# syncdoth/face_mask_inpaint

Measured on AMD Instinct MI355X. Metric: train images/sec at 256x256 bs=8 per GPU (PICNet-ref train step), higher is better.
Workload: dtype f32; 1 GPU; train_reference_fill.py PICNet-ref 256x256 fp32, bs=8 per GPU, synthetic CelebA-HQ-shaped batch + random binary_map (BASELINE configs[1]); global_batch=8, parallelism=dp1

## Files before the change

face_mask_inpaint_amd/_lib.py:

```python
from __future__ import annotations

import ctypes as C
import os

_HERE = os.path.dirname(os.path.abspath(__file__))
LIB_PATH = os.path.join(_HERE, "csrc", "libfmi_hip.so")

c_f = C.c_void_p
i32, i64, f32, vp = C.c_int, C.c_int64, C.c_float, C.c_void_p


class ConvDesc(C.Structure):

    _fields_ = [(n, C.c_int) for n in ("N", "H", "W", "C", "OH", "OW", "K", "x_cstride", "y_cstride", "kh", "kw", "stride", "pad", "pad_mode", "dil")] + [("w3", C.c_void_p), ("x3", C.c_void_p), ("y3", C.c_void_p)]


class WeightEntry(C.Structure):
    _fields_ = [("w", vp), ("u", vp), ("v", vp), ("wf", vp), ("wt", vp), ("sigma", vp), ("rows", i32), ("C", i32), ("taps", i32), ("iters", i32), ("wf3", vp), ("wt3", vp)]


class WeightGradEntry(C.Structure):
    _fields_ = [("w", vp), ("u", vp), ("v", vp), ("sigma", vp), ("dwf", vp), ("dw", vp), ("rows", i32), ("C", i32), ("taps", i32), ("pad_", i32)]


# ... 82 lines not shown
    "fmi_add_bcast_f32": [vp, vp, vp, i32, i64, i32, vp],
    "fmi_scale_channels_bwd_f32": [vp, vp, vp, vp, vp, vp, i64, i32, i64, i32, vp],
    "fmi_subsample_bf16": [vp, vp, i32, i32, i32, i32, i32, i32, vp],
    "fmi_scale_channels_add_f32": [vp, vp, vp, vp, i32, i64, i32, vp],
    "fmi_instnorm_bwd_apply_add_f32": [vp, vp, vp, vp, vp, vp, vp, vp, vp, vp, i32, i32, i32, f32, vp],
    "fmi_copy_channels_f32": [vp, vp, i64, i32, i32, i32, i32, i32, vp],
    "fmi_l2norm_rows_f32": [vp, vp, vp, i64, i32, f32, vp],
    "fmi_l2norm_rows_bwd_f32": [vp, vp, vp, vp, i64, i32, f32, vp],
    "fmi_lpips_layer_f32": [vp, vp, vp, vp, i64, i32, f32, vp],
    "fmi_lpips_layer_bwd_f32": [vp, vp, vp, vp, vp, vp, i64, i32, f32, vp],
    "fmi_maxpool2_bwd_f32": [vp, vp, vp, i32, i32, i32, i32, vp],
    "fmi_resize_bilinear_f32": [vp, vp, i32, i32, i32, i32, i32, i32, vp, vp, vp],
    "fmi_resize_bilinear_bwd_f32": [vp, vp, i32, i32, i32, i32, i32, i32, vp, vp],
    "fmi_instnorm_stats_f32": [vp, vp, vp, i32, i32, i32, f32, vp, i64, vp],
    "fmi_batchnorm_running_update_f32": [vp, vp, vp, vp, vp, i32, i64, f32, f32, vp],
    "fmi_instnorm_apply_f32": [vp, vp, vp, vp, vp, i32, i32, i32, f32, vp],
    "fmi_instnorm_bwd_reduce_f32": [vp, vp, vp, vp, vp, vp, i32, i32, i32, f32, vp, i64, vp],
    "fmi_instnorm_bwd_apply_f32": [vp, vp, vp, vp, vp, vp, vp, vp, vp, i32, i32, i32, f32, vp],
    "fmi_reduce_loss_f32": [i32, vp, vp, i64, f32, f32, vp, vp],
    "fmi_reduce_loss_bwd_f32": [i32, vp, vp, i64, f32, f32, vp, vp, vp],
    "fmi_ssim_f32": [vp, vp, vp, i32, i32, i32, i32, i32, vp, vp],
    "fmi_cx_channel_mean_f32": [vp, vp, i64, i32, vp],
    "fmi_cx_normalise_f32": [vp, vp, vp, vp, i64, i32, vp],
    "fmi_cx_normalise_bwd_f32": [vp, vp, vp, vp, i64, i32, vp],
    "fmi_cx_rows_f32": [vp, vp, vp, vp, vp, i32, i32, f32, vp],
    "fmi_cx_cols_f32": [vp, vp, vp, i32, i32, vp],
    "fmi_cx_loss_f32": [vp, vp, vp, i32, i32, f32, vp],
    "fmi_cx_bwd_f32": [vp, vp, vp, vp, vp, vp, vp, vp, vp, i32, i32, f32, f32, vp],
    "fmi_adam_step_f32": [vp, i32, i64, f32, f32, f32, f32, f32, i32, vp],
    "fmi_adam_step_dev_f32": [vp, i32, f32, f32, f32, f32, f32, vp, vp],
    "fmi_adam_step_dev_guarded_f32": [vp, i32, f32, f32, f32, f32, f32, vp, vp, vp],
    "fmi_ranger_step_f32": [vp, i32, f32, f32, f32, f32, f32, f32, i32, f32, i32, vp],
    "fmi_upfirdn2d_f32": [vp, vp, vp, i32, i32, i32, i32, i32, i32, i32, i32, i32, i32, i32, i32, i32, vp],
    "fmi_upfirdn2d_bf16": [vp, vp, vp, i32, i32, i32, i32, i32, i32, i32, i32, i32, i32, i32, i32, i32, vp],
    "fmi_fused_bias_act_f32": [vp, vp, vp, vp, i64, i32, i32, i32, i32, f32, f32, vp],
    "fmi_fused_bias_act_bf16": [vp, vp, vp, vp, i64, i32, i32, i32, i32, f32, f32, vp],
    "fmi_scale_channels_f32": [vp, vp, vp, i32, i64, i32, vp],
    "fmi_scale_channels_gs_f32": [vp, vp, vp, vp, i64, i32, i64, i32, vp],
    "fmi_sqsum_last_f32": [vp, vp, i64, i32, vp],
    "fmi_sqsum_last_bwd_f32": [vp, vp, vp, i64, i32, vp],
    "fmi_noise_bias_act_bwd_f32": [vp, vp, vp, vp, vp, i64, i32, f32, f32, vp],
    "fmi_upfirdn2d_nhwc_f32": [vp, vp, vp, i32, i32, i32, i32, i32, i32, i32, i32, i32, i32, i32, i32, i32, i32, vp],
    "fmi_prelu_f32": [vp, vp, vp, i64, i32, vp],
    "fmi_prelu_bwd_f32": [vp, vp, vp, vp, vp, vp, i64, i64, i32, vp],
    "fmi_subsample_f32": [vp, vp, i32, i32, i32, i32, i32, i32, vp],
    "fmi_bias_grad_nchw_f32": [vp, i32, i32, i64, vp, vp],
    "fmi_bias_grad_nchw_bf16": [vp, i32, i32, i64, vp, vp],
    "fmi_noise_bias_act_f32": [vp, vp, vp, vp, vp, i64, i32, f32, f32, vp],
}

STATUS = {0: "ok", 1: "bad argument", 2: "unsupported shape/mode", 3: "kernel launch failed"}


PREDICATES = {"fmi_debug_bf16_tile": [i32], "fmi_set_deterministic": [i32], "fmi_get_deterministic": [], "fmi_conv2d_thin_supported": [PD], "fmi_conv2d_bf16_supported": [PD], "fmi_conv2d_thin_lrelu_supported": [PD]}


class FmiError(RuntimeError):
    pass


class Library:

    def __init__(self, path: str = LIB_PATH, strict: bool = True):
        if not os.path.exists(path):
            raise FmiError(
                f"{path} not found: build the HIP extension first (python -c 'import __graft_entry__ as g; g.build()'). "
                "There is no CPU fallback."
            )
        self.path = path
        self.cdll = C.CDLL(path)
        self.missing = []
        for name, argtypes in SIGNATURES.items():
            try:
                fn = getattr(self.cdll, name)
            except AttributeError:
                self.missing.append(name)
                continue
            fn.argtypes = argtypes
            fn.restype = C.c_int
            setattr(self, name[4:], self._checked(name, fn))
        for name, argtypes in PREDICATES.items():
            try:
                fn = getattr(self.cdll, name)
            except AttributeError:
                self.missing.append(name)
                continue
            fn.argtypes = argtypes
            fn.restype = C.c_int
            setattr(self, name[4:], fn)
        if strict and self.missing:
            raise FmiError(f"{path} lacks symbols {self.missing}")

    @staticmethod
    def _checked(name, fn):
        def call(*args):
            rc = fn(*args)
            if rc != 0:
                raise FmiError(f"{name} failed: {STATUS.get(rc, rc)}")

        call.__name__ = name
        return call


_LIB = None


def lib() -> Library:
# ... 5 lines not shown
```

face_mask_inpaint_amd/csrc/conv.hip:

```cpp
#include "gemm_core.h"
#include "conv3x3.h"
#include "conv_p3.h"
#include "convt3x3.h"

static bool aligned16(const void* p) { return ((uintptr_t)p & 15) == 0; }
static bool ep_scalar() {
  static const bool v = getenv("FMI_EP_SCALAR") != nullptr;
  return v;
}

static int check_desc(const fmi_conv_desc* d) {
  if (!d) return FMI_ERR_BAD_ARG;
  if (d->N <= 0 || d->H <= 0 || d->W <= 0 || d->C <= 0 || d->K <= 0 || d->kh <= 0 || d->kw <= 0 || d->stride <= 0 ||
      d->pad < 0 || d->x_cstride < d->C || d->y_cstride < d->K)
    return FMI_ERR_BAD_ARG;
  const int pe = d->pad, dl = d->dil > 1 ? d->dil : 1;
  if (d->dil < 0 || (dl > 1 && d->pad_mode)) return FMI_ERR_BAD_ARG;
  if (d->OH != (d->H + 2 * pe - dl * (d->kh - 1) - 1) / d->stride + 1 || d->OW != (d->W + 2 * pe - dl * (d->kw - 1) - 1) / d->stride + 1)
    return FMI_ERR_BAD_ARG;
  if (d->OH <= 0 || d->OW <= 0) return FMI_ERR_BAD_ARG;
  if (d->pad_mode == 1 && (d->pad >= d->H || d->pad >= d->W)) return FMI_ERR_UNSUPPORTED;
  if (d->pad_mode != 0 && d->pad_mode != 1) return FMI_ERR_UNSUPPORTED;
  if ((int64_t)d->N * d->H * d->W > 0x7fffffffLL / 2 || (int64_t)d->kh * d->kw * d->C > 0x3fffffffLL) return FMI_ERR_UNSUPPORTED;
  return FMI_OK;
}

static ConvGeom fwd_geom(const fmi_conv_desc* d, const float* x, int n_eff) {
  ConvGeom g{};
  g.N = n_eff; g.IH = d->H; g.IW = d->W; g.C = d->C; g.cstride = d->x_cstride;
  g.GH = d->OH; g.GW = d->OW; g.S = d->stride;
  const int dl = d->dil > 1 ? d->dil : 1;
  g.nty = d->kh; g.ntx = d->kw; g.dy0 = -d->pad; g.dx0 = -d->pad; g.ystep = dl; g.xstep = dl;
  g.kh0 = 0; g.kw0 = 0; g.khstep = 1; g.kwstep = 1; g.kw = d->kw;
  g.pad_mode = d->pad_mode;
  g.vec = (d->C % 4 == 0) && (d->x_cstride % 4 == 0) && aligned16(x);
  g.dGW = make_fastdiv(g.GW); g.dG = make_fastdiv(g.GH * g.GW); g.dC = make_fastdiv(g.C); g.dntx = make_fastdiv(g.ntx);
  g.img_bs = (int64_t)d->H * d->W * d->x_cstride;
  return g;
}

#ifndef FMI_HOST_EMU
__global__ void __launch_bounds__(256) conv_split_init_kernel(float* __restrict__ y, const float* __restrict__ bias,
                                                             const float* __restrict__ res, int K, int cstride, int64_t total) {
  for (int64_t i = (int64_t)blockIdx.x * 256 + threadIdx.x; i < total; i += (int64_t)gridDim.x * 256) {
    const int k = (int)(i % K);
    const int64_t o = (i / K) * cstride + k;
    float v = bias ? bias[k] : 0.f;
    if (res) v += res[o];
    y[o] = v;
  }
}
#endif

static int conv_ksplit(int64_t M, int N, int K) {
#ifdef FMI_HOST_EMU
  return 1;
// ... 296 lines not shown
        continue;
      }
#endif
      rc = launch_gemm(la, lb, ep, g.Mdim(), d->C, g.Kdim(), batch_w, 1, (hipStream_t)stream);
      if (rc) return rc;
    }
  }
  return FMI_OK;
}
extern "C" int fmi_conv2d_dgrad_f32(const fmi_conv_desc* d, const float* dy, const float* wt, const float* bias,
                                    const float* residual, float* dx, int batch_w, int64_t w_bstride, void* stream) {
  return dgrad_impl(d, dy, wt, bias, residual, nullptr, 0.f, dx, batch_w, w_bstride, stream);
}
extern "C" int fmi_conv_transpose2d_pair_f32(const fmi_conv_desc* d, const float* x1, const float* x2, int K2, const void* w3b,
                                             const float* bias, float* y, void* stream) {
  int rc = check_desc(d);
  if (rc) return rc;
  if (!x1 || !x2 || !w3b || !d->w3 || !y || K2 <= 0) return FMI_ERR_BAD_ARG;
#ifndef FMI_HOST_EMU
  const uint16_t* w3 = (FMI_X6 && d->K % 16 == 0 && aligned16(d->w3)) ? (const uint16_t*)d->w3 : nullptr;
  if (!convt3x3_eligible(d, x1, w3) || (K2 & 15) || !aligned16(x2) || !aligned16(w3b) || d->pad_mode != 0 || d->x3) return FMI_ERR_UNSUPPORTED;
  CT3Args ca{};
  ca.x = x1; ca.w3 = w3; ca.x2 = x2; ca.w3b = (const uint16_t*)w3b; ca.Cred2 = K2; ca.cs2 = K2;
  ca.N = d->N; ca.H = d->OH; ca.W = d->OW; ca.Cred = d->K; ca.cs = d->y_cstride; ca.Nout = d->C;
  ca.dW = make_fastdiv(d->OW); ca.dHW = make_fastdiv(d->OH * d->OW);
  ConvEp ep{y, bias, nullptr, d->OH, d->OW, 2, 0, 0, d->H, d->W, d->x_cstride, 0, ca.dW, ca.dHW, (int64_t)d->H * d->W * d->x_cstride};
  ep.vec = !ep_scalar() && d->C % 4 == 0 && d->x_cstride % 4 == 0 && aligned16(y) && aligned16(bias);
  ca.ep = ep;
  return launch_convt3x3(ca, d->N * d->OH * d->OW, (hipStream_t)stream);
#else
  return FMI_ERR_UNSUPPORTED;
#endif
}
extern "C" int fmi_conv2d_dgrad_masked_f32(const fmi_conv_desc* d, const float* dy, const float* wt, const float* mask, float mask_slope,
                                           float* dx, void* stream) {
  if (!mask) return FMI_ERR_BAD_ARG;
  return dgrad_impl(d, dy, wt, nullptr, nullptr, mask, mask_slope, dx, 1, 0, stream);
}

extern "C" int fmi_conv2d_dgrad_masked_add_f32(const fmi_conv_desc* d, const float* dy, const float* wt, const float* mask, float mask_slope,
                                               const float* gadd, float* dx, void* stream) {
  if (!mask || !gadd) return FMI_ERR_BAD_ARG;
  return dgrad_impl(d, dy, wt, nullptr, gadd, mask, mask_slope, dx, 1, 0, stream);
}

extern "C" int fmi_conv2d_wgrad_f32(const fmi_conv_desc* d, const float* x, const float* dy, float* dwf, float* dbias,
                                    int batch_w, int64_t w_bstride, void* stream) {
  int rc = check_desc(d);
  if (rc) return rc;
  if (!x || !dy || !dwf || batch_w < 1) return FMI_ERR_BAD_ARG;
  if (batch_w > 1 && batch_w != d->N) return FMI_ERR_BAD_ARG;
#ifndef FMI_HOST_EMU
  if (batch_w == 1 && fmi_conv2d_thin_supported(d) && aligned16(x)) return fmi_conv2d_thin_wgrad_f32(d, x, dy, dwf, dbias, stream);
#endif
#ifndef FMI_HOST_EMU
  static const bool wg3_off = getenv("FMI_WG3_OFF") != nullptr || getenv("FMI_P3_OFF") != nullptr;
  if (!wg3_off && FMI_X6 && batch_w == 1 && !dbias && wgrad_p3_ok(d, d->x3, d->y3))
    return launch_wgrad_p3(d, (const uint16_t*)d->x3, (const uint16_t*)d->y3, dwf, (hipStream_t)stream);
#endif
  const int n_eff = batch_w > 1 ? 1 : d->N;
  ConvGeom g = fwd_geom(d, x, n_eff);
  const bool fuse_bias = dbias && batch_w == 1 && (g.Kdim() % 4 == 0);
  if (dbias && !fuse_bias) return FMI_ERR_UNSUPPORTED;
  const int ones_row = fuse_bias ? g.Kdim() : -1;
  const int Mg = g.Kdim() + (fuse_bias ? 1 : 0), Ng = d->K, Kg = g.Mdim();
  WgradAX la{x, g, ones_row};
  DenseX lb{dy, (int64_t)d->y_cstride, (int64_t)d->OH * d->OW * d->y_cstride, Ng, Kg,
            (d->K % 4 == 0) && (d->y_cstride % 4 == 0) && aligned16(dy)};
  WgradEp ep{dwf, g, d->K, w_bstride, dbias, ones_row};
  const int64_t tiles = ceil_div64(Mg, 128) * ceil_div64(Ng, Ng <= 32 ? 32 : (Ng <= 64 ? 64 : 128));
  int64_t ksplit = 2048 / (tiles * batch_w);
  const int64_t kmax = Kg / 512;
  if (ksplit > kmax) ksplit = kmax;
  if (ksplit < 1) ksplit = 1;
  static const int wks_dbg = getenv("FMI_WKS") ? atoi(getenv("FMI_WKS")) : 0;
  if (wks_dbg > 0) ksplit = wks_dbg;
  if (fmi_det()) ksplit = 1;
  if (ksplit * batch_w > 65535) ksplit = 65535 / batch_w;
  return launch_gemm(la, lb, ep, Mg, Ng, Kg, batch_w, (int)ksplit, (hipStream_t)stream);
}

#ifndef FMI_HOST_EMU
__global__ void __launch_bounds__(256) bias_grad_vec_f64_kernel(const float* __restrict__ g, int64_t rows, int K4, float* __restrict__ dbias) {
  __shared__ double part[256][4];
  const int cg = threadIdx.x % K4, rl = threadIdx.x / K4, RL = 256 / K4;
  double s[4] = {0, 0, 0, 0};
  for (int64_t r = rl; r < rows; r += RL) {
    const float4 v = reinterpret_cast<const float4*>(g)[r * K4 + cg];
    s[0] += v.x, s[1] += v.y, s[2] += v.z, s[3] += v.w;
  }
#pragma unroll
  for (int e = 0; e < 4; ++e) part[threadIdx.x][e] = s[e];
  __syncthreads();
  if (threadIdx.x < K4) {
    double t[4] = {0, 0, 0, 0};
    for (int l = 0; l < RL; ++l)
#pragma unroll
      for (int e = 0; e < 4; ++e) t[e] += part[l * K4 + threadIdx.x][e];
#pragma unroll
    for (int e = 0; e < 4; ++e) atomicAdd(dbias + 4 * threadIdx.x + e, (float)t[e]);
  }
}
__global__ void __launch_bounds__(256) bias_grad_vec_kernel(const float* __restrict__ g, int64_t rows, int K4,
                                                            float* __restrict__ dbias, int64_t rows_per_block) {
  __shared__ float4 part[256];
  const int cg = threadIdx.x % K4, rl = threadIdx.x / K4, RL = 256 / K4;
  const int64_t r0 = (int64_t)blockIdx.x * rows_per_block;
  int64_t r1 = r0 + rows_per_block;
  if (r1 > rows) r1 = rows;
  float4 s = make_float4(0.f, 0.f, 0.f, 0.f);
  int64_t r = r0 + rl;
  for (; r + 3 * RL < r1; r += 4 * RL) {
    const float4 v0 = reinterpret_cast<const float4*>(g)[r * K4 + cg];
    const float4 v1 = reinterpret_cast<const float4*>(g)[(r + RL) * K4 + cg];
    const float4 v2 = reinterpret_cast<const float4*>(g)[(r + 2 * RL) * K4 + cg];
    const float4 v3 = reinterpret_cast<const float4*>(g)[(r + 3 * RL) * K4 + cg];
    s.x += (v0.x + v1.x) + (v2.x + v3.x);
    s.y += (v0.y + v1.y) + (v2.y + v3.y);
    s.z += (v0.z + v1.z) + (v2.z + v3.z);
    s.w += (v0.w + v1.w) + (v2.w + v3.w);
  }
  for (; r < r1; r += RL) {
    const float4 v = reinterpret_cast<const float4*>(g)[r * K4 + cg];
    s.x += v.x; s.y += v.y; s.z += v.z; s.w += v.w;
  }
  part[threadIdx.x] = s;
  __syncthreads();
  if (threadIdx.x < K4) {
    float4 t = part[threadIdx.x];
    for (int l = 1; l < RL; ++l) {
      const float4 v = part[l * K4 + threadIdx.x];
      t.x += v.x; t.y += v.y; t.z += v.z; t.w += v.w;
// ... 76 lines not shown
```

face_mask_inpaint_amd/functional.py:

```python
from __future__ import annotations

import ctypes as C
import math
import os
from typing import List, Optional, Sequence, Tuple

import torch

from . import _lib
from ._lib import ConvDesc, FmiError

EW_LRELU, EW_LRELU_BWD, EW_TANH_BWD, EW_ADD, EW_SCALE, EW_AXPY, EW_MUL, EW_RELU_BWD_OUT, EW_SOFTPLUS, EW_SOFTPLUS_BWD, EW_SUB, EW_RSQRT, EW_RSQRT_BWD, EW_SIGMOID, EW_SIGMOID_BWD = range(15)
ACT_NONE, ACT_TANH, ACT_RELU = 0, 1, 2

ATTN_CHUNK_BYTES = 96 * 1024 * 1024

PROFILE = None


class _prof:
    def __init__(self, tag, flops):
        self.tag, self.flops = tag, flops

    def __enter__(self):
# ... 293 lines not shown
        if gy is None:
            return (gpass,) + (None,) * 15
        kh, kw, stride, pad, pad_mode, act = ctx.cfg
        gy = gy.contiguous()
        if act and not ctx.skip_act_bwd:
            gy = _act_bwd(gy, y, act)
        n, h, w, c = x.shape
        k = wf.shape[2]
        gx = gwf = gb = gres = None
        masked = False
        dil = ctx.dil
        gb_of_split = [] if (ctx.has[0] and ctx.needs_input_grad[2]) else None
        if ctx.needs_input_grad[0]:
            d0, _, _ = conv_desc(n, h, w, c, k, kh, kw, stride, pad, pad_mode, dil=dil)
            if pad_mode == 1 and lib.conv2d_thin_supported(C.byref(d0)):
                gx = torch.empty_like(x)
                with _prof(f"conv_dgrad|{n}x{h}x{w} {c}->{k} k{kh}s{stride}", 2.0 * gy.numel() * c * kh * kw):
                    lib.conv2d_thin_dgrad_f32(C.byref(d0), _p(gy), _p(ctx.wt), _p(gx), _st())
            elif pad_mode == 1:
                hp, wp = h + 2 * pad, w + 2 * pad
                d, _, _ = conv_desc(n, hp, wp, c, k, kh, kw, stride, 0, w3=ctx.wt3)
                gpad = torch.empty((n, hp, wp, c), device=x.device, dtype=torch.float32)
                with _prof(f"conv_dgrad|{n}x{h}x{w} {c}->{k} k{kh}s{stride}", 2.0 * gy.numel() * c * kh * kw):
                    lib.conv2d_dgrad_f32(C.byref(d), _p(gy), _p(ctx.wt), None, None, _p(gpad), 1, 0, _st())
                gx = torch.empty_like(x)
                lib.reflect_pad_fold_f32(_p(gpad), _p(gx), n, h, w, c, pad, _st())
            else:
                oh_, ow_ = gy.shape[1], gy.shape[2]
                gy3 = p3_of(gy, colsum=gb_of_split) if (ctx.wt3 is not None and p3_wanted(n * oh_ * ow_, k, c, kh * kw)) else None
                d, _, _ = conv_desc(n, h, w, c, k, kh, kw, stride, pad, dil=dil, w3=ctx.wt3, x3=gy3)
                gx = torch.empty_like(x)
                with _prof(f"conv_dgrad|{n}x{h}x{w} {c}->{k} k{kh}s{stride}", 2.0 * gy.numel() * c * kh * kw):
                    if ctx.in_slope is not None and gpass is not None:
                        lib.conv2d_dgrad_masked_add_f32(C.byref(d), _p(gy), _p(ctx.wt), _p(x), ctx.in_slope, _p(gpass.contiguous()), _p(gx), _st())
                        masked, gpass = True, None
                    elif ctx.in_slope is not None:
                        lib.conv2d_dgrad_masked_f32(C.byref(d), _p(gy), _p(ctx.wt), _p(x), ctx.in_slope, _p(gx), _st())
                        masked = True
                    elif gpass is not None:
                        lib.conv2d_dgrad_f32(C.byref(d), _p(gy), _p(ctx.wt), None, _p(gpass.contiguous()), _p(gx), 1, 0, _st())
                        gpass = None
                    else:
                        lib.conv2d_dgrad_f32(C.byref(d), _p(gy), _p(ctx.wt), None, None, _p(gx), 1, 0, _st())
            if ctx.in_slope is not None and not masked:
                gx = eltwise(EW_LRELU_BWD, gx, x, ctx.in_slope)
            if gpass is not None:
                gx = eltwise(EW_ADD, gx, gpass.contiguous())
        elif gpass is not None:
            gx = gpass
        if ctx.needs_input_grad[1]:
            d, _, _ = conv_desc(n, h, w, c, k, kh, kw, stride, pad, pad_mode, dil=dil)
            gwf = _zeros_like(wf)
            want_gb = ctx.has[0] and ctx.needs_input_grad[2]
            if ctx.x3 is not None and pad_mode == 0 and c % 32 == 0 and k % 16 == 0 and p3_wanted(gy.numel() // k, c, k, kh * kw):
                gy3 = p3_of(gy, colsum=gb_of_split)
                if gy3 is not None:
                    d.w3 = None
                    d.x3, d.y3 = ctx.x3.data_ptr(), gy3.data_ptr()
                    want_gb_fused = False
                else:
                    want_gb_fused = want_gb
            else:
                want_gb_fused = want_gb
            fuse = want_gb_fused and (kh * kw * c) % 4 == 0
            if fuse:
                gb = _zeros(k, x.device, torch.float32)
            with _prof(f"conv_wgrad|{n}x{h}x{w} {c}->{k} k{kh}s{stride}", 2.0 * gy.numel() * c * kh * kw):
                lib.conv2d_wgrad_f32(C.byref(d), _p(x), _p(gy), _p(gwf), _p(gb) if fuse else None, 1, 0, _st())
        if ctx.has[0] and ctx.needs_input_grad[2] and gb is None:
            if gb_of_split:
                gb = gb_of_split[0]
            else:
                gb = _zeros(k, x.device, torch.float32)
                lib.bias_grad_f32(_p(gy), gy.numel() // k, k, k, _p(gb), _st())
        if ctx.has[1] and ctx.needs_input_grad[3]:
            gres = gy
        return gx, gwf, gb, gres, None, None, None, None, None, None, None, None, None, None, None, None


class _ThinConvLReLU(torch.autograd.Function):

    @staticmethod
    def forward(ctx, x, wf, bias, wt, slope, pad_mode, act):
        _chk(x, wf, bias)
        n, h, w, c = x.shape
        k = wf.shape[2]
        d, oh, ow = conv_desc(n, h, w, c, k, 3, 3, 1, 1, pad_mode)
        y = torch.empty((n, oh, ow, k), device=x.device, dtype=torch.float32)
        with _prof(f"conv_fwd|{n}x{h}x{w} {c}->{k} k3s1", 2.0 * n * oh * ow * k * c * 9):
            _L().conv2d_thin_lrelu_fwd_f32(C.byref(d), _p(x), slope, _p(wf), _p(bias), _p(y), act, _st())
        ctx.save_for_backward(x, wf, y if act else None)
        ctx.wt, ctx.cfg, ctx.has_b = wt, (slope, pad_mode, act), bias is not None
        return y

    @staticmethod
    def backward(ctx, gy):
        lib = _L()
        x, wf, y = ctx.saved_tensors
        slope, pad_mode, act = ctx.cfg
        gy = gy.contiguous()
        if act:
            gy = _act_bwd(gy, y, act)
        n, h, w, c = x.shape
        k = wf.shape[2]
        d, _, _ = conv_desc(n, h, w, c, k, 3, 3, 1, 1, pad_mode)
        gx = gwf = gb = None
        if ctx.needs_input_grad[0]:
# ... 282 lines not shown
def _bias_grad_of(gy, cb):
    m = _BIAS_GRAD_MEMO
    if m[0] is not None and m[0].data_ptr() == gy.data_ptr() and m[0].shape == gy.shape and m[0]._version == gy._version and m[2] == gy._version:
        return m[1].clone()
    gb = _zeros(cb, gy.device, torch.float32)
    _L().bias_grad_f32(_p(gy), gy.numel() // cb, cb, cb, _p(gb), _st())
    m[:] = [gy, gb, gy._version]
    return gb.clone()


class _ConvTranspose2d(torch.autograd.Function):

    @staticmethod
    def forward(ctx, x, wf, bias, residual, wt, kh, kw, stride, pad, out_pad, w3=(None, None)):
        _chk(x, wf, bias, residual)
        lib = _L()
        n, h, w, cs = x.shape
        cb = wf.shape[1]
        H = (h - 1) * stride - 2 * pad + kh + out_pad
        W = (w - 1) * stride - 2 * pad + kw + out_pad
        x3 = p3_of(x) if (w3[1] is not None and p3_wanted(n * h * w, cs, cb, kh * kw)) else None
        d, oh, ow = conv_desc(n, H, W, cb, cs, kh, kw, stride, pad, w3=w3[1], x3=x3)
        ctx.wf3 = w3[0]
        ctx.x3 = x3
        if (oh, ow) != (h, w):
            raise FmiError("unsupported ConvTranspose2d geometry")
        y = torch.empty((n, H, W, cb), device=x.device, dtype=torch.float32)
        with _prof(f"convT_fwd|{n}x{h}x{w} {cs}->{cb}", 2.0 * x.numel() * cb * kh * kw):
            lib.conv2d_dgrad_f32(C.byref(d), _p(x), _p(wt), _p(bias), _p(residual), _p(y), 1, 0, _st())
        ctx.save_for_backward(x, wf)
        ctx.cfg, ctx.has, ctx.HW = (kh, kw, stride, pad), (bias is not None, residual is not None), (H, W)
        return y

    @staticmethod
    def backward(ctx, gy):
        lib = _L()
        x, wf = ctx.saved_tensors
        kh, kw, stride, pad = ctx.cfg
        H, W = ctx.HW
        gy = gy.contiguous()
        n, h, w, cs = x.shape
        cb = wf.shape[1]
        d, _, _ = conv_desc(n, H, W, cb, cs, kh, kw, stride, pad, w3=ctx.wf3)
        gx = gwf = gb = gres = None
        gb_of_split = [] if (ctx.has[0] and ctx.needs_input_grad[2]) else None
        if ctx.needs_input_grad[0]:
            gx = torch.empty_like(x)
            gy3 = p3_of(gy, colsum=gb_of_split) if (ctx.wf3 is not None and p3_wanted(n * H * W, cb, cs, kh * kw)) else None
            d0, _, _ = conv_desc(n, H, W, cb, cs, kh, kw, stride, pad, w3=ctx.wf3, x3=gy3)
            with _prof(f"convT_dgrad|{n}x{h}x{w} {cs}->{cb}", 2.0 * x.numel() * cb * kh * kw):
                lib.conv2d_fwd_f32(C.byref(d0), _p(gy), _p(wf), None, None, _p(gx), 0, 1, 0, _st())
        if ctx.needs_input_grad[1]:
            gwf = _zeros_like(wf)
            if ctx.x3 is not None and cb % 32 == 0 and cs % 16 == 0:
                gy3 = p3_of(gy, colsum=gb_of_split)
                if gy3 is not None:
                    d.x3, d.y3 = gy3.data_ptr(), ctx.x3.data_ptr()
            with _prof(f"convT_wgrad|{n}x{h}x{w} {cs}->{cb}", 2.0 * x.numel() * cb * kh * kw):
                lib.conv2d_wgrad_f32(C.byref(d), _p(gy), _p(x), _p(gwf), None, 1, 0, _st())
        if ctx.has[0] and ctx.needs_input_grad[2]:
            gb = gb_of_split[0] if gb_of_split else _bias_grad_of(gy, cb)
        if ctx.has[1] and ctx.needs_input_grad[3]:
            gres = gy
        return gx, gwf, gb, gres, None, None, None, None, None, None, None


class _ConvTransposePair(torch.autograd.Function):

    @staticmethod
    def forward(ctx, x1, wf1, wt1, x2, wf2, wt2, bias, w3_1, w3_2):
        _chk(x1, wf1, x2, wf2, bias)
        n, h, w, cs1 = x1.shape
        cs2, cb = x2.shape[3], wf1.shape[1]
        H, W = 2 * h, 2 * w
        d, oh, ow = conv_desc(n, H, W, cb, cs1, 3, 3, 2, 1, w3=w3_1[1])
        y = torch.empty((n, H, W, cb), device=x1.device, dtype=torch.float32)
        with _prof(f"convT_pair_fwd|{n}x{h}x{w} {cs1}+{cs2}->{cb}", 2.0 * (x1.numel() + x2.numel()) * cb * 9):
            _L().conv_transpose2d_pair_f32(C.byref(d), _p(x1), _p(x2), cs2, C.c_void_p(w3_2[1].data_ptr()), _p(bias), _p(y), _st())
        ctx.save_for_backward(x1, wf1, x2, wf2)
        ctx.w3s, ctx.HW, ctx.has_bias = (w3_1, w3_2), (H, W), bias is not None
        return y

    @staticmethod
    def backward(ctx, gy):
        import types

        x1, wf1, x2, wf2 = ctx.saved_tensors
        gy = gy.contiguous()
        outs = []
        for x, wf, w3, ix, iw in ((x1, wf1, ctx.w3s[0], 0, 1), (x2, wf2, ctx.w3s[1], 3, 4)):
            ns = types.SimpleNamespace(saved_tensors=(x, wf), cfg=(3, 3, 2, 1), has=(False, False), HW=ctx.HW, wf3=w3[0], x3=None,
                                       needs_input_grad=(ctx.needs_input_grad[ix], ctx.needs_input_grad[iw]) + (False,) * 9)
            outs.append(_ConvTranspose2d.backward(ns, gy)[:2])
        gb = _bias_grad_of(gy, gy.shape[-1]) if (ctx.has_bias and ctx.needs_input_grad[6]) else None
        return outs[0][0], outs[0][1], None, outs[1][0], outs[1][1], None, gb, None, None


def conv_transpose2d_pair_ok(x1, pw1: PackedWeight, x2, pw2: PackedWeight) -> bool:
    if x1.dtype != torch.float32 or x2.dtype != torch.float32 or not x1.is_cuda or x1.shape[:3] != x2.shape[:3]:
        return False
    if os.environ.get("FMI_CT3_OFF"):
        return False
    n, h, w, cs1 = x1.shape
    cs2, cb = x2.shape[3], pw1.wf.shape[1]
    return (pw1.kh == 3 and pw1.kw == 3 and pw2.kh == 3 and pw2.kw == 3 and pw2.wf.shape[1] == cb and cb <= 64 and cb % 4 == 0 and cs1 % 16 == 0 and
            cs2 % 16 == 0 and n * h * w >= 32768 and pw1.w3[1] is not None and pw2.w3[1] is not None and x1.is_contiguous() and x2.is_contiguous() and
            not p3_wanted(n * h * w, cs1, cb, 9))
# ... 1356 lines not shown
```

include/fmi_hip.h:

```cpp
#ifndef FMI_HIP_H
#define FMI_HIP_H

#include <stdint.h>

#ifdef __cplusplus
extern "C" {
#endif

typedef enum {
  FMI_OK = 0,
  FMI_ERR_BAD_ARG = 1,
  FMI_ERR_UNSUPPORTED = 2,
  FMI_ERR_LAUNCH = 3
} fmi_status;

const char* fmi_status_string(int status);
int fmi_version(void);
int fmi_set_deterministic(int on);
int fmi_get_deterministic(void);

int fmi_debug_bf16_tile(int mode);

int fmi_gemm_f32(const float* A, const float* B, float* C, int M, int N, int K,
                 int64_t sa_m, int64_t sa_k, int64_t sb_k, int64_t sb_n, int64_t sc_m, int64_t sc_n,
                 int batch, int64_t sa_b, int64_t sb_b, int64_t sc_b,
                 float alpha, float beta, const float* bias, void* stream);

typedef struct {
  int N, H, W, C;
  int OH, OW, K;
  int x_cstride;
  int y_cstride;
  int kh, kw, stride, pad;
  int pad_mode;
  int dil;
  const void* w3;
  const void* x3;
  void* y3;
} fmi_conv_desc;

int fmi_resample_u8(const uint8_t* in, uint8_t* out, int N, int in_h, int in_w, int C, int out_len, int axis, int row0, int rows,
                    const int32_t* bounds, const int32_t* kk, int ksize, void* stream);
int fmi_gather_u8_i64(const uint8_t* in, int64_t* out, int N, int in_h, int in_w, int out_h, int out_w, const int32_t* ytab,
                      const int32_t* xtab, void* stream);
int fmi_u8_lut_chw_f32(const uint8_t* in, const float* lut256, float* out, int N, int H, int W, int C, void* stream);

int fmi_split3_f32(const float* x, void* x3, float* y, int64_t pixels, int C, int op, float p0, void* stream);
int fmi_merge3_f32(const void* x3, float* y, int64_t pixels, int C, void* stream);
int fmi_split3_colsum_f32(const float* x, void* x3, float* colsum, int64_t pixels, int C, void* stream);

int fmi_conv2d_fwd_f32(const fmi_conv_desc* d, const float* x, const float* wf, const float* bias,
                       const float* residual, float* y, int act, int batch_w, int64_t w_bstride, void* stream);
int fmi_conv_transpose2d_pair_f32(const fmi_conv_desc* d, const float* x1, const float* x2, int K2, const void* w3b, const float* bias,
                                  float* y, void* stream);
int fmi_conv2d_dgrad_f32(const fmi_conv_desc* d, const float* dy, const float* wt, const float* bias,
                         const float* residual, float* dx, int batch_w, int64_t w_bstride, void* stream);
int fmi_conv2d_dgrad_masked_f32(const fmi_conv_desc* d, const float* dy, const float* wt, const float* mask, float mask_slope, float* dx,
                                void* stream);
int fmi_conv2d_dgrad_masked_add_f32(const fmi_conv_desc* d, const float* dy, const float* wt, const float* mask, float mask_slope,
                                    const float* gadd, float* dx, void* stream);
int fmi_conv2d_wgrad_f32(const fmi_conv_desc* d, const float* x, const float* dy, float* dwf, float* dbias,
                         int batch_w, int64_t w_bstride, void* stream);
int fmi_conv2d_thin_supported(const fmi_conv_desc* d);
int fmi_conv2d_thin_fwd_f32(const fmi_conv_desc* d, const float* x, const float* wf, const float* bias,
                            const float* residual, float* y, int act, void* stream);
int fmi_conv2d_thin_dgrad_f32(const fmi_conv_desc* d, const float* dy, const float* wt, float* dx, void* stream);
int fmi_conv2d_thin_wgrad_f32(const fmi_conv_desc* d, const float* x, const float* dy, float* dwf, float* dbias, void* stream);
int fmi_conv2d_thin_lrelu_supported(const fmi_conv_desc* d);
int fmi_conv2d_thin_lrelu_fwd_f32(const fmi_conv_desc* d, const float* x, float in_slope, const float* wf, const float* bias, float* y, int act,
                                  void* stream);
int fmi_conv2d_thin_lrelu_dgrad_f32(const fmi_conv_desc* d, const float* dy, const float* wt, const float* x, float in_slope, float* dx,
                                    void* stream);
int fmi_conv2d_thin_lrelu_wgrad_f32(const fmi_conv_desc* d, const float* x, float in_slope, const float* dy, float* dwf, float* dbias,
                                    void* stream);
int fmi_conv2d_thin_input_dgrad_f32(const fmi_conv_desc* d, const float* dy, const float* wt, float* dx, void* stream);
int fmi_conv2d_bf16_supported(const fmi_conv_desc* d);
int fmi_conv2d_fwd_bf16(const fmi_conv_desc* d, const uint16_t* x, const uint16_t* wnk, const float* colscale, uint16_t* y, float* ws,
                        int64_t ws_floats, void* stream);
int fmi_conv2d_fwd_act_bf16(const fmi_conv_desc* d, const uint16_t* x, const uint16_t* wnk, const float* colscale, const float* noise,
                            const float* nw, const float* bias, float slope, float gain, uint16_t* y, void* stream);
int fmi_conv2d_dgrad_bf16(const fmi_conv_desc* d, const uint16_t* dy, const uint16_t* wck, const float* colscale, uint16_t* dx, float* ws,
                          int64_t ws_floats, void* stream);
int fmi_conv2d_wgrad_bf16(const fmi_conv_desc* d, const uint16_t* x, const uint16_t* dy, float* dwf, void* stream);
int fmi_pack_weight_bf16(const float* src_tab, uint16_t* dst_bta, int T, int A, int B, void* stream);
int fmi_scale_channels_bf16(const uint16_t* x, const float* s, uint16_t* y, int N, int64_t P, int C, void* stream);
int fmi_scale_channels_gs_bf16(const uint16_t* g, const uint16_t* x, float* gs, float* ws, int64_t ws_floats, int N, int64_t P, int C,
                               void* stream);
int fmi_noise_bias_act_bf16(const uint16_t* x, const float* bias, const float* noise, const float* nw, uint16_t* y, int64_t pixels, int C,
                            float alpha, float scale, void* stream);
int fmi_noise_bias_act_bwd_bf16(const uint16_t* g, const uint16_t* y, const float* noise, uint16_t* gx, float* gnw, float* gbias,
                                float* ws, int64_t ws_floats, int64_t pixels, int C, float alpha, float scale, void* stream);
int fmi_upfirdn2d_nhwc_bf16(const uint16_t* in, const float* kernel, uint16_t* out, int N, int in_h, int in_w, int C, int kh, int kw,
                            int up_x, int up_y, int down_x, int down_y, int pad_x0, int pad_x1, int pad_y0, int pad_y1, void* stream);
int fmi_blur_act_bf16(const uint16_t* in, const float* kernel, uint16_t* out, int N, int in_h, int in_w, int C, int pad_x0, int pad_x1,
                      int pad_y0, int pad_y1, const float* colscale, const float* noise, const float* nw, const float* bias, float slope,
                      float gain, int separable, void* stream);
int fmi_styled_out_bwd_bf16(const uint16_t* g, const uint16_t* y, const float* noise, const float* colscale, const float* nw,
                            const float* bias, uint16_t* t, float* gd, float* gbias, float* gnw, float* ws, int64_t ws_floats, float* sums,
                            int N, int64_t P, int C, float slope, float gain, void* stream);
int fmi_torgb_fwd_bf16(const uint16_t* x, const float* w, const float* s, const float* bias, const float* skip, float* out, int N,
                       int64_t P, int C, void* stream);
int fmi_torgb_bwd_bf16(const uint16_t* x, const float* w, const float* s, const float* g, uint16_t* gx, float* ws, int64_t ws_floats,
                       float* gw, float* gs, float* gbias, int N, int64_t P, int C, void* stream);

int fmi_bias_grad_f32(const float* g, int64_t rows, int K, int cstride, float* dbias, void* stream);
int fmi_reflect_pad_fold_f32(const float* gpad, float* gx, int N, int H, int W, int C, int pad, void* stream);

typedef struct {
  const float* w;
  float* u;
  float* v;
  float* wf;
  float* wt;
  float* sigma;
  int rows, C, taps;
// ... 188 lines not shown
```

Measured before the change: 102.4 images/s.

## Add dedicated thin 3x3 weight-gradient kernel with implicit im2col and bf16x3 MFMA

Adds a specialized wgrad kernel for 3x3 pad-1 convolutions with small channel counts (at most 128, not both above 64) on large stride-1 maps. It streams input rows and output-gradient tiles through a double or quad-buffered LDS ring, splits fp32 into three bf16 parts on the fly, and accumulates with MFMA using transposed LDS reads. Bias gradients are fused in, and partial results are combined across workgroups with atomics. This path is taken ahead of the generic GEMM and the precomputed-split p3 paths, which the Python side now skips for these shapes to avoid producing split copies of the output gradient. The cost is nondeterministic atomic accumulation and more code paths to keep correct.

```diff
diff --git a/face_mask_inpaint_amd/_lib.py b/face_mask_inpaint_amd/_lib.py
--- a/face_mask_inpaint_amd/_lib.py
+++ b/face_mask_inpaint_amd/_lib.py
@@ -158,7 +158,7 @@
 STATUS = {0: "ok", 1: "bad argument", 2: "unsupported shape/mode", 3: "kernel launch failed"}
 
 
-PREDICATES = {"fmi_debug_bf16_tile": [i32], "fmi_set_deterministic": [i32], "fmi_get_deterministic": [], "fmi_conv2d_thin_supported": [PD], "fmi_conv2d_bf16_supported": [PD], "fmi_conv2d_thin_lrelu_supported": [PD]}
+PREDICATES = {"fmi_debug_bf16_tile": [i32], "fmi_set_deterministic": [i32], "fmi_get_deterministic": [], "fmi_conv2d_thin_supported": [PD], "fmi_conv2d_bf16_supported": [PD], "fmi_conv2d_thin_lrelu_supported": [PD], "fmi_conv2d_wgrad_thin3x3_supported": [PD]}
 
 
 class FmiError(RuntimeError):
diff --git a/face_mask_inpaint_amd/csrc/conv.hip b/face_mask_inpaint_amd/csrc/conv.hip
--- a/face_mask_inpaint_amd/csrc/conv.hip
+++ b/face_mask_inpaint_amd/csrc/conv.hip
@@ -2,6 +2,7 @@
 #include "conv3x3.h"
 #include "conv_p3.h"
 #include "convt3x3.h"
+#include "wgrad_thin3x3.h"
 
 static bool aligned16(const void* p) { return ((uintptr_t)p & 15) == 0; }
 static bool ep_scalar() {
@@ -404,6 +405,7 @@
   if (batch_w > 1 && batch_w != d->N) return FMI_ERR_BAD_ARG;
 #ifndef FMI_HOST_EMU
   if (batch_w == 1 && fmi_conv2d_thin_supported(d) && aligned16(x)) return fmi_conv2d_thin_wgrad_f32(d, x, dy, dwf, dbias, stream);
+  if (batch_w == 1 && wgrad_thin3x3_ok(d, x, dy)) return launch_wgrad_thin3x3(d, x, dy, dwf, dbias, (hipStream_t)stream);
 #endif
 #ifndef FMI_HOST_EMU
   static const bool wg3_off = getenv("FMI_WG3_OFF") != nullptr || getenv("FMI_P3_OFF") != nullptr;
@@ -430,6 +432,13 @@
   if (fmi_det()) ksplit = 1;
   if (ksplit * batch_w > 65535) ksplit = 65535 / batch_w;
   return launch_gemm(la, lb, ep, Mg, Ng, Kg, batch_w, (int)ksplit, (hipStream_t)stream);
+}
+extern "C" int fmi_conv2d_wgrad_thin3x3_supported(const fmi_conv_desc* d) {
+#ifndef FMI_HOST_EMU
+  return d && check_desc(d) == FMI_OK && wgrad_thin3x3_shape_ok(d) ? 1 : 0;
+#else
+  return 0;
+#endif
 }
 
 #ifndef FMI_HOST_EMU
diff --git a/face_mask_inpaint_amd/csrc/wgrad_thin3x3.h b/face_mask_inpaint_amd/csrc/wgrad_thin3x3.h
--- /dev/null
+++ b/face_mask_inpaint_amd/csrc/wgrad_thin3x3.h
@@ -0,0 +1,268 @@
+#pragma once
+#ifndef FMI_HOST_EMU
+#include "x6.h"
+
+struct WgtArgs {
+  const float* x;
+  const float* dy;
+  float* dwf;
+  float* dbias;
+  int H, W, C, OH, OW, K;
+  int rows, nbands;
+  int nchunks, cpw, nxs;
+  int kblocks, nblk;
+};
+
+template <int S, int TC, int TK>
+struct WgtCfg {
+  static constexpr int NW = 3 * TC * TK, NT = 64 * NW;
+  static constexpr int CB = 32 * TC, KB = 32 * TK;
+  static constexpr int P = S == 1 ? 2 : 1;
+  static constexpr int XPX = S == 1 ? 18 : 33;
+  static constexpr int XP = S == 1 ? 18 : 34;
+  static constexpr int XPC = TC * XP * 64;
+  static constexpr int XSR = 3 * XPC;
+  static constexpr int NXS = S == 1 ? 4 : 3;
+  static constexpr int XSLOT = S * XSR;
+  static constexpr int DPC = TK * 1024;
+  static constexpr int DOFF = NXS * XSLOT;
+  static constexpr int LDS = DOFF + 2 * 3 * DPC;
+  static constexpr int NXU = S * XPX * TC * 4, NDU = 16 * TK * 4;
+  static constexpr int NU = (NXU + NDU + NT - 1) / NT;
+  static_assert(LDS <= 65536, "static LDS");
+  static_assert(16 * KB * 4 <= LDS, "bias reduction fits");
+};
+
+typedef short wgt_s16x4 __attribute__((ext_vector_type(4)));
+
+template <int S, int TC, int TK>
+__global__ void __launch_bounds__(192 * TC * TK, 3) wgrad_thin3x3_kernel(WgtArgs a) {
+  using G = WgtCfg<S, TC, TK>;
+  constexpr int P = G::P, NU = G::NU;
+  __shared__ __attribute__((aligned(1024))) unsigned char lds[G::LDS];
+  const int tid = threadIdx.x, lane = tid & 63, wid = tid >> 6;
+  const int l31 = lane & 31, lh = lane >> 5;
+
+  int u = blockIdx.x;
+  const int blk = u % a.nblk;
+  u /= a.nblk;
+  const int xs = u % a.nxs;
+  u /= a.nxs;
+  const int band = u % a.nbands, n = u / a.nbands;
+  const int cblk = blk / a.kblocks, kblk = blk - cblk * a.kblocks;
+  const int c0 = cblk * G::CB, k0 = kblk * G::KB;
+  const int j0 = band * a.rows, j1 = min(j0 + a.rows, a.OH);
+  const int q0 = xs * a.cpw, q1 = min(q0 + a.cpw, a.nchunks);
+  const int spc = j1 - j0 + P;
+  const int T = (q1 - q0) * spc;
+  const float* xn = a.x + (int64_t)n * a.H * a.W * a.C;
+  const float* dyn = a.dy + (int64_t)n * a.OH * a.OW * a.K;
+
+  int u_kind[NU], u_sr[NU], u_px[NU], u_ch[NU], u_lds[NU];
+#pragma unroll
+  for (int i = 0; i < NU; ++i) {
+    const int q = tid + i * G::NT;
+    u_kind[i] = 0, u_sr[i] = 0, u_px[i] = 0, u_ch[i] = 0, u_lds[i] = 0;
+    if (q < G::NXU) {
+      const int sr = q / (G::XPX * TC * 4), rem = q - sr * (G::XPX * TC * 4);
+      const int px = rem / (TC * 4), c8 = rem - px * (TC * 4);
+      const int pos = S == 1 ? px : ((px & 1) ? 17 + (px >> 1) : (px >> 1));
+      u_kind[i] = c0 + 8 * c8 < a.C ? 1 : 0;
+      u_sr[i] = sr, u_px[i] = px, u_ch[i] = c0 + 8 * c8;
+      u_lds[i] = sr * G::XSR + (c8 >> 2) * (G::XP * 64) + pos * 64 + (c8 & 3) * 16;
+    } else if (q < G::NXU + G::NDU) {
+      const int r = q - G::NXU, px = r / (TK * 4), k8 = r - px * (TK * 4);
+      u_kind[i] = k0 + 8 * k8 < a.K ? 2 : 0;
+      u_px[i] = px, u_ch[i] = k0 + 8 * k8;
+      u_lds[i] = G::DOFF + (k8 >> 2) * 1024 + px * 64 + (k8 & 3) * 16;
+    }
+  }
+  float v[NU][8];
+  float bsum[NU][8];
+#pragma unroll
+  for (int i = 0; i < NU; ++i)
+#pragma unroll
+    for (int e = 0; e < 8; ++e) bsum[i][e] = 0.f;
+
+  auto load = [&](int qi, int s) __attribute__((always_inline)) {
+    const int j = j0 - P + s, x0 = qi * 16;
+#pragma unroll
+    for (int i = 0; i < NU; ++i) {
+      bool ok = false;
+      const float* p = xn;
+      if (u_kind[i] == 1) {
+        const int row = S * j + 2 - S + u_sr[i], px = S * x0 - 1 + u_px[i];
+        ok = (unsigned)row < (unsigned)a.H && (unsigned)px < (unsigned)a.W;
+        p = xn + ((int64_t)row * a.W + px) * a.C + u_ch[i];
+      } else if (u_kind[i] == 2) {
+        const int px = x0 + u_px[i];
+        ok = s >= P && px < a.OW;
+        p = dyn + ((int64_t)j * a.OW + px) * a.K + u_ch[i];
+      }
+      float4 f0 = make_float4(0.f, 0.f, 0.f, 0.f), f1 = f0;
+      if (ok) {
+        f0 = reinterpret_cast<const float4*>(p)[0];
+        f1 = reinterpret_cast<const float4*>(p)[1];
+      }
+      v[i][0] = f0.x, v[i][1] = f0.y, v[i][2] = f0.z, v[i][3] = f0.w;
+      v[i][4] = f1.x, v[i][5] = f1.y, v[i][6] = f1.z, v[i][7] = f1.w;
+    }
+  };
+  auto store = [&](int xsl, int dsl) __attribute__((always_inline)) {
+#pragma unroll
+    for (int i = 0; i < NU; ++i) {
+      if (u_kind[i] == 0) continue;
+      bf16x8_t pc[3];
+      split3_bf16(v[i], pc);
+      const bool isx = u_kind[i] == 1;
+      const int base = u_lds[i] + (isx ? xsl * G::XSLOT : dsl * 3 * G::DPC);
+      const int pstride = isx ? G::XPC : G::DPC;
+#pragma unroll
+      for (int k = 0; k < 3; ++k) *reinterpret_cast<bf16x8_t*>(lds + base + k * pstride) = pc[k];
+      if (!isx) {
+#pragma unroll
+        for (int e = 0; e < 8; ++e) bsum[i][e] += v[i][e];
+      }
+    }
+  };
+
+  const int ky = wid % 3, ct = (wid / 3) / TK, kt = (wid / 3) - ct * TK;
+  const int i16 = lane & 15;
+  const uint32_t lcol = (uint32_t)(32 * ((lane >> 4) & 1) + 8 * (i16 & 3));
+  const int prow = 8 * lh + (i16 >> 2);
+  const uint32_t lds0 = (uint32_t)(uintptr_t)(__attribute__((address_space(3))) unsigned char*)lds;
+  const uint32_t lane_off = lds0 + (uint32_t)(prow * 64) + lcol;
+  typedef __attribute__((address_space(3))) wgt_s16x4* lp;
+  auto tr2 = [&](uint32_t a0) __attribute__((always_inline)) {
+    union {
+      wgt_s16x4 h[2];
+      bf16x8_t v;
+    } r;
+    r.h[0] = __builtin_amdgcn_ds_read_tr16_b64_v4i16((lp)(uintptr_t)a0);
+    r.h[1] = __builtin_amdgcn_ds_read_tr16_b64_v4i16((lp)(uintptr_t)(a0 + 256u));
+    return r.v;
+  };
+  f32x16 acc[3];
+#pragma unroll
+  for (int kx = 0; kx < 3; ++kx)
+#pragma unroll
+    for (int r = 0; r < 16; ++r) acc[kx][r] = 0.f;
+  auto compute = [&](int cur, int dcur) __attribute__((always_inline)) {
+    int xsl, sub;
+    if constexpr (S == 1) {
+      xsl = (cur + 2 + ky) & 3, sub = 0;
+    } else {
+      xsl = ky == 0 ? (cur == 0 ? 2 : cur - 1) : cur, sub = ky == 1 ? 0 : 1;
+    }
+    const uint32_t xb = lane_off + (uint32_t)(xsl * G::XSLOT + sub * G::XSR + ct * (G::XP * 64));
+    const uint32_t db = lane_off + (uint32_t)(G::DOFF + dcur * 3 * G::DPC + kt * 1024);
+    bf16x8_t pb[3];
+#pragma unroll
+    for (int pc = 0; pc < 3; ++pc) pb[pc] = tr2(db + (uint32_t)(pc * G::DPC));
+#pragma unroll
+    for (int kx = 0; kx < 3; ++kx) {
+      const int sh = S == 1 ? kx : (kx == 1 ? 17 : kx >> 1);
+      bf16x8_t pa[3];
+#pragma unroll
+      for (int pc = 0; pc < 3; ++pc) pa[pc] = tr2(xb + (uint32_t)(pc * G::XPC + sh * 64));
+      acc[kx] = mfma_x6(pa, pb, acc[kx]);
+    }
+  };
+
+  load(q0, 0);
+  store(0, 0);
+  __syncthreads();
+  int qi = q0, s = 0, cur = 0, dcur = 0;
+  for (int t = 0; t < T; ++t) {
+    int qn = qi, sn = s + 1;
+    if (sn == spc) sn = 0, ++qn;
+    const bool more = t + 1 < T;
+    if (more) load(qn, sn);
+    if (s >= P) compute(cur, dcur);
+    const int curn = cur + 1 == G::NXS ? 0 : cur + 1;
+    if (more) store(curn, dcur ^ 1);
+    __syncthreads();
+    qi = qn, s = sn, cur = curn, dcur ^= 1;
+  }
+
+#pragma unroll
+  for (int kx = 0; kx < 3; ++kx) {
+#pragma unroll
+    for (int r = 0; r < 16; ++r) {
+      const int c = c0 + ct * 32 + (r & 3) + 8 * (r >> 2) + 4 * lh, k = k0 + kt * 32 + l31;
+      if (c < a.C && k < a.K) atomicAdd(a.dwf + ((int64_t)(ky * 3 + kx) * a.C + c) * a.K + k, acc[kx][r]);
+    }
+  }
+  if (a.dbias && cblk == 0) {
+    float* red = reinterpret_cast<float*>(lds);
+#pragma unroll
+    for (int i = 0; i < NU; ++i) {
+      const int q = tid + i * G::NT;
+      if (q >= G::NXU && q < G::NXU + G::NDU) {
+        const int r = q - G::NXU, px = r / (TK * 4), k8 = r - px * (TK * 4);
+#pragma unroll
+        for (int e = 0; e < 8; ++e) red[px * G::KB + 8 * k8 + e] = bsum[i][e];
+      }
+    }
+    __syncthreads();
+    if (tid < G::KB && k0 + tid < a.K) {
+      float sum = 0.f;
+      for (int px = 0; px < 16; ++px) sum += red[px * G::KB + tid];
+      atomicAdd(a.dbias + k0 + tid, sum);
+    }
+  }
+}
+
+static bool wgrad_thin3x3_shape_ok(const fmi_conv_desc* d) {
+  const char* off = getenv("FMI_WGT_OFF");
+  if (off && off[0] && off[0] != '0') return false;
+  if (fmi_det() || d->kh != 3 || d->kw != 3 || d->pad != 1 || d->pad_mode != 0 || d->dil > 1) return false;
+  if (!(d->stride == 1 || (d->stride == 2 && d->H == 2 * d->OH && d->W == 2 * d->OW))) return false;
+  if (d->C % 16 || d->K % 16 || d->C > 128 || d->K > 128 || (d->C > 64 && d->K > 64)) return false;
+  if (d->x_cstride != d->C || d->y_cstride != d->K || (int64_t)d->N * d->OH * d->OW >= 0x7fffffffLL) return false;
+  const char* all = getenv("FMI_WGT_ALL");
+  if (all && all[0] && all[0] != '0') return true;
+  return d->stride == 1 && (int64_t)d->OH * d->OW >= 65536;
+}
+static bool wgrad_thin3x3_ok(const fmi_conv_desc* d, const float* x, const float* dy) {
+  return wgrad_thin3x3_shape_ok(d) && !((uintptr_t)x & 15) && !((uintptr_t)dy & 15);
+}
+
+static int launch_wgrad_thin3x3(const fmi_conv_desc* d, const float* x, const float* dy, float* dwf, float* dbias, hipStream_t st) {
+  const int S = d->stride;
+  const int TC = (S == 1 && d->C > 32) ? 2 : 1;
+  const int TK = d->K > 32 ? 2 : 1;
+  WgtArgs a{};
+  a.x = x, a.dy = dy, a.dwf = dwf, a.dbias = dbias;
+  a.H = d->H, a.W = d->W, a.C = d->C, a.OH = d->OH, a.OW = d->OW, a.K = d->K;
+  const int cblocks = (int)ceil_div64(d->C, 32 * TC);
+  a.kblocks = (int)ceil_div64(d->K, 32 * TK);
+  a.nblk = cblocks * a.kblocks;
+  static const int rows_dbg = getenv("FMI_WGT_ROWS") ? atoi(getenv("FMI_WGT_ROWS")) : 0;
+  static const int wgs_dbg = getenv("FMI_WGT_WGS") ? atoi(getenv("FMI_WGT_WGS")) : 0;
+  a.rows = rows_dbg > 0 ? rows_dbg : 8;
+  if (a.rows > d->OH) a.rows = d->OH;
+  a.nbands = (int)ceil_div64(d->OH, a.rows);
+  a.nchunks = (int)ceil_div64(d->OW, 16);
+  const int64_t want = wgs_dbg > 0 ? wgs_dbg : 512;
+  const int64_t units = (int64_t)d->N * a.nbands * a.nblk;
+  a.cpw = a.nchunks;
+  while (a.cpw > 1 && units * ceil_div64(a.nchunks, a.cpw) < want) a.cpw = (a.cpw + 1) / 2;
+  a.nxs = (int)ceil_div64(a.nchunks, a.cpw);
+  const int64_t nwg = units * a.nxs;
+  if (nwg > 0x7fffffffLL) return FMI_ERR_UNSUPPORTED;
+#define WGT_LAUNCH(S_, TC_, TK_) \
+  hipLaunchKernelGGL((wgrad_thin3x3_kernel<S_, TC_, TK_>), dim3((unsigned)nwg), dim3(WgtCfg<S_, TC_, TK_>::NT), 0, st, a)
+  if (S == 1) {
+    if (TC == 1 && TK == 1) WGT_LAUNCH(1, 1, 1);
+    else if (TC == 1) WGT_LAUNCH(1, 1, 2);
+    else if (TK == 1) WGT_LAUNCH(1, 2, 1);
+    else WGT_LAUNCH(1, 2, 2);
+  } else {
+    if (TK == 1) WGT_LAUNCH(2, 1, 1);
+    else WGT_LAUNCH(2, 1, 2);
+  }
+#undef WGT_LAUNCH
+  return fmi_launch_status();
+}
+#endif
diff --git a/face_mask_inpaint_amd/functional.py b/face_mask_inpaint_amd/functional.py
--- a/face_mask_inpaint_amd/functional.py
+++ b/face_mask_inpaint_amd/functional.py
@@ -369,7 +369,8 @@
             d, _, _ = conv_desc(n, h, w, c, k, kh, kw, stride, pad, pad_mode, dil=dil)
             gwf = _zeros_like(wf)
             want_gb = ctx.has[0] and ctx.needs_input_grad[2]
-            if ctx.x3 is not None and pad_mode == 0 and c % 32 == 0 and k % 16 == 0 and p3_wanted(gy.numel() // k, c, k, kh * kw):
+            if ctx.x3 is not None and pad_mode == 0 and c % 32 == 0 and k % 16 == 0 and p3_wanted(gy.numel() // k, c, k, kh * kw) and \
+                    not lib.conv2d_wgrad_thin3x3_supported(C.byref(d)):
                 gy3 = p3_of(gy, colsum=gb_of_split)
                 if gy3 is not None:
                     d.w3 = None
@@ -758,7 +759,7 @@
                 lib.conv2d_fwd_f32(C.byref(d0), _p(gy), _p(wf), None, None, _p(gx), 0, 1, 0, _st())
         if ctx.needs_input_grad[1]:
             gwf = _zeros_like(wf)
-            if ctx.x3 is not None and cb % 32 == 0 and cs % 16 == 0:
+            if ctx.x3 is not None and cb % 32 == 0 and cs % 16 == 0 and not lib.conv2d_wgrad_thin3x3_supported(C.byref(d)):
                 gy3 = p3_of(gy, colsum=gb_of_split)
                 if gy3 is not None:
                     d.x3, d.y3 = gy3.data_ptr(), ctx.x3.data_ptr()
diff --git a/include/fmi_hip.h b/include/fmi_hip.h
--- a/include/fmi_hip.h
+++ b/include/fmi_hip.h
@@ -61,6 +61,7 @@
                                     const float* gadd, float* dx, void* stream);
 int fmi_conv2d_wgrad_f32(const fmi_conv_desc* d, const float* x, const float* dy, float* dwf, float* dbias,
                          int batch_w, int64_t w_bstride, void* stream);
+int fmi_conv2d_wgrad_thin3x3_supported(const fmi_conv_desc* d);
 int fmi_conv2d_thin_supported(const fmi_conv_desc* d);
 int fmi_conv2d_thin_fwd_f32(const fmi_conv_desc* d, const float* x, const float* wf, const float* bias,
                             const float* residual, float* y, int act, void* stream);
```

Measured after the change: 103.9 images/s, median of 6. 1.01x the previous value.
